# mo-hanxuan/FEMcy

Hardware: AMD Instinct MI355X
Metric: CG iters/sec + element-stiffness assemblies/sec, 1M C3D4 elems, 1/2/4/8 GPU (higher is better)
Workload: dtype f64; 1 GPU; twist plate C3D4 96x12x144 cells, 995328 elements, 548535 DOF (BASELINE configs[2] at N=1, configs[3] at N=8), state S1 (t=0.05), step = assemble K + Dirichlet + 1000 PCG iterations; elements_per_gpu=995328, parallelism=single GPU, launcher=single process

## Files before the change

femcy_amd/backend.py:

```python
from __future__ import annotations

import ctypes as C
import os
from typing import Optional, Sequence

import numpy as np

_HERE = os.path.dirname(os.path.abspath(__file__))
LIB_PATH = os.environ.get("FEMCY_HIP_LIB") or os.path.join(_HERE, "libfemcy_hip.so")
CPU_LIB_PATH = os.environ.get("FEMCY_CPU_LIB") or os.path.join(_HERE, "libfemcy_cpu.so")


def default_backend() -> str:
    kind = os.environ.get("FEMCY_BACKEND", "hip").lower()
    if kind not in ("hip", "cpu"):
        raise FemcyError(f"FEMCY_BACKEND={kind!r}: expected 'hip' or 'cpu'")
    return kind

VEC_DOF, VEC_RHS, VEC_RESIDUAL, VEC_FORCE, VEC_DU, VEC_DOF_OLD, VEC_X, VEC_TMP0, VEC_TMP1 = range(9)
GP_DSDX, GP_VOL, GP_F, GP_SIGMA, GP_STRAIN, GP_MISES, GP_ENERGY = range(7)
OPT_ASSEMBLY, OPT_PCG_POLL, OPT_TIMING, OPT_SPMV_VARIANT, OPT_EW_GRID, OPT_PCG_GRAPH, OPT_SELL_SIGMA = range(7)
OPT_TANGENT = 7
OPT_EXCHANGE = 8
OPT_PCG_STORAGE_ORDER = 13
OPT_PCG_FUSED_UPDATE = 15
OPT_SPMV_FOOTPRINT = 16
OPT_DIRECT_MAX_BYTES = 17
OPT_NODE_ORDER = 14
OPT_PCG_PERSIST = 11
OPT_PCG_PERSIST_MULTI = 12
OPT_PCG_SMALL = 10
TUNE_PERSIST_VARIANT = 109
TUNE_SKIP_OCCUPANCY_CHECK = 111
TUNE_BARRIER_SPIN_LIMIT = 112
TUNE_PERSIST_L2_ROWS = 113
TUNE_SPMV_WG_PER_XCD = 101
TUNE_SPMV_ROT = 119
TUNE_PAIRS = 117
TUNE_DIRECT_UPDATE = 115
TUNE_PERSIST_MAX_MB = 114
OPT_OVERLAP = 9
ASM_GATHER, ASM_ATOMIC, ASM_ROWS, ASM_AUTO, ASM_GATHER_SYM, ASM_GATHER_SYM_ROWSUM, ASM_ROWS2, ASM_ROWS4, ASM_PAIRS = 0, 1, 2, 3, 4, 5, 6, 8, 9
ASM_ROWS3 = 7

EXPORTS = [
    "femcy_ctx_create", "femcy_ctx_destroy", "femcy_last_error", "femcy_version", "femcy_set_option", "femcy_sync",
    "femcy_set_mesh", "femcy_set_element", "femcy_set_material", "femcy_build_pattern", "femcy_get_pattern_info",
    "femcy_get_assembly_used",
    "femcy_vec_upload", "femcy_vec_download", "femcy_vec_fill", "femcy_vec_copy", "femcy_vec_scatter",
    "femcy_vec_sub", "femcy_vec_axpy", "femcy_vec_scale", "femcy_vec_norm", "femcy_vec_absmax",
# ... 510 lines not shown
```

femcy_amd/csrc/ctx.hpp:

```cpp
#pragma once
#include <hip/hip_runtime.h>
#include <stdint.h>
#include <stdlib.h>
#include <mutex>
#include <string>
#include <vector>
#include "../../include/femcy.h"

namespace femcy {

void set_error(const char* fmt, ...);

#define FEMCY_HIP(call)                                                                         \
    do {                                                                                        \
        hipError_t _e = (call);                                                                 \
        if (_e != hipSuccess) {                                                                 \
            femcy::set_error("%s failed: %s (%s:%d)", #call, hipGetErrorString(_e), __FILE__, __LINE__); \
            return FEMCY_EHIP;                                                                  \
        }                                                                                       \
    } while (0)

inline hipError_t dfill_sync(void* p, int value, size_t bytes) {
    if (!bytes) return hipSuccess;
#ifdef FEMCY_TEST_LATE_FILL
// ... 168 lines not shown
    double* d_val_scratch = nullptr;
    int64_t scratch_cap = 0;

    hipGraphExec_t pcg_graph = nullptr;
    const double* pcg_graph_x = nullptr;
    int pcg_graph_iters = 0, pcg_graph_g = 0, pcg_graph_np1 = 0;
    int opt_graph = 1;
    int opt_persist = 1;
    int64_t persist_max_bytes = (int64_t)1 << 40;
    int opt_persist_rj = 4;
    int opt_persist_wgs = 0;
    int opt_persist_l2rows = 1;
    int opt_persist_variant = -1;
    int opt_persist_dbg = 0;
    int opt_persist_lds = -1;
    int persist_cus = 0;
    bool persist_failed = false;
    bool small_failed = false;
    int opt_skip_occupancy = 0;
    uint32_t barrier_spin_limit = 1u << 20;
    int32_t* d_persist_assign = nullptr;
    std::vector<int64_t> persist_assign_key;
    int64_t pattern_serial = 0;
    double* d_persist = nullptr;
    int64_t persist_cap = 0;
    int32_t* d_bcolp = nullptr;
    int64_t bcolp_serial = -1;
    int opt_spmv_fp = 0;
    uint16_t* d_lcol = nullptr;
    int32_t* d_fp_ptr = nullptr;
    int32_t* d_fp = nullptr;
    int32_t fp_cap = 0;
    int64_t fp_serial = -1;
    int opt_fused_update = 0;
    bool fused_failed = false;
    double* d_fused = nullptr;
    int opt_pos_space = 1;
// ... 166 lines not shown
```

femcy_amd/csrc/femcy_api.cpp:

```cpp
#include <algorithm>
#include <cmath>
#include <cstdarg>
#include <chrono>
#include <cstdio>
#include <cstring>
#include "ctx.hpp"
#include "direct.hpp"

namespace femcy {

static thread_local char g_err[1024] = "";

void set_error(const char* fmt, ...) {
    va_list ap;
    va_start(ap, fmt);
    vsnprintf(g_err, sizeof(g_err), fmt, ap);
    va_end(ap);
}

template <class T>
static int dev_alloc(T** p, size_t count, bool zero = true) {
    if (*p) {
        (void)hipFree(*p);
        *p = nullptr;
// ... 291 lines not shown
            break;
        case FEMCY_OPT_EXCHANGE:
            FEMCY_REQUIRE(value == 0 || value == 1, "exchange: 0 (all-reduce) or 1 (neighbour send/recv)");
            FEMCY_REQUIRE(value == 0 || c->d_if_ptr, "femcy_comm_set_neighbours must come first");
            c->exchange = (int)value;
            break;
        case FEMCY_OPT_PCG_PERSIST:
            FEMCY_REQUIRE(value >= 0 && value <= 2, "persistent PCG: 0 (off), 1 (auto) or 2 (whenever the slices fit)");
            c->opt_persist = (int)value;
            c->persist_failed = false;
            break;
        case FEMCY_TUNE_PERSIST_LDS_ROWS:
            FEMCY_REQUIRE(value >= -1 && value <= 64, "resident block rows out of range");
            c->opt_persist_lds = (int)value;
            break;
        case FEMCY_TUNE_SPMV_KEEP:
            FEMCY_REQUIRE(value >= -1 && value <= 1000, "per-mille out of range (-1 = auto)");
            c->opt_spmv_keep = (int)value;
            if (c->have_pattern) {
                pcg_graph_reset(c);
                spmv_split(c);
            }
            break;
        case FEMCY_TUNE_SMALL_REG_ROWS:
            FEMCY_REQUIRE(value >= -1 && value <= 64, "register-resident rows out of range");
            c->opt_small_rr = (int)value;
            break;
        case FEMCY_TUNE_PERSIST_WGS:
            FEMCY_REQUIRE(value >= 0 && value <= 4096, "workgroup count out of range");
            c->opt_persist_wgs = (int)value;
// ... 42 lines not shown
        case FEMCY_TUNE_PERSIST_VARIANT:
            FEMCY_REQUIRE(value >= -1 && value <= 15 && (value < 8 || value == 14), "variant bits: -1 (default), 0..7 or 14");
            c->opt_persist_variant = (int)value;
            break;
        case FEMCY_TUNE_PERSIST_PROBE:
#ifdef FEMCY_PERSIST_PROBE
            c->opt_persist_dbg = (int)value;
            break;
#else
            FEMCY_REQUIRE(value == 0 || value == 16, "option 106: the work-skipping timing switches (bits 0-3) exist only in a "
                                                     "-DFEMCY_PERSIST_PROBE build; 16 (no prefetch during the barriers) is always available");
            c->opt_persist_dbg = (int)value;
            break;
#endif
        case FEMCY_TUNE_PERSIST_REG_ROWS:
#ifdef FEMCY_PERSIST_PIPE
            FEMCY_REQUIRE(value == 0 || value == 2 || value == 4 || value == 5, "register-resident block rows: 0, 2, 4 or 5");
#else
            FEMCY_REQUIRE(value == 0 || value == 4 || value == 5, "register-resident block rows: 0, 4 or 5");
#endif
            c->opt_persist_rj = (int)value;
            break;
        case FEMCY_OPT_PCG_SMALL:
            FEMCY_REQUIRE(value == 0 || value == 1, "small-system PCG: 0 (off) or 1 (auto)");
            c->opt_small = (int)value;
            c->small_failed = false;
            break;
        case FEMCY_OPT_OVERLAP:
            FEMCY_REQUIRE(value == 0 || value == 1, "overlap: 0 (one stream) or 1 (exchange overlapped with the interior product)");
            c->opt_overlap = (int)value;
            break;
        case FEMCY_OPT_TANGENT:
            FEMCY_REQUIRE(value == 0 || value == 1, "tangent: 0 (reference) or 1 (consistent)");
            c->opt_tangent = (int)value;
            break;
// ... 1011 lines not shown
```

femcy_amd/csrc/kernels_pcg_persist.hip:

```cpp
#include <algorithm>
#include <cmath>
#include <type_traits>
#include <vector>
#include "ctx.hpp"
#include "wave_reduce.hpp"
#include "granule.hpp"

#if defined(__HIP_DEVICE_COMPILE__) && !defined(__gfx950__) && !defined(__gfx942__)
#error "k_pcg_persist: the sc1-only hand-off protocol is validated for gfx942 / gfx950 only"
#endif

namespace femcy {

namespace {

constexpr int PBS = 256;
constexpr int PNX = 8;
constexpr int CH = 4;
constexpr int V_NT = 1, V_A2A = 2, V_WIDE = 4, V_INBAND = 8;
constexpr unsigned SENT_HI = 0xFFFBADD0u, SENT_LO = 0x5E471E70u;

#ifdef FEMCY_PERSIST_PROBE
#define PDBG(a_, bit_) ((a_).dbg & (bit_))
#else
#define PDBG(a_, bit_) false
#endif

struct PersistPcg {
    const int32_t* slice_len;
    const int64_t* slice_off;
    const int32_t* bcol;
    const int32_t* node_of;
    const int32_t* assign;
    const double* vals;
    const double* b;
    const double* M;
    double* x;
    double* dbuf;
    double* part1;
    double* part2;
    double* slots;
    unsigned int* xc;
    unsigned int* top;
    PcgState* st;
    int32_t npad, maxit, lds_rows, dbg, l2_rows;
    uint32_t spin_limit;
    uint32_t xspin_limit;
    double eps;
    unsigned long long* mbox;
    unsigned long long* const* peer;
    const int32_t* mr_tab;
    const uint8_t* owner;
    int32_t rank, nranks, nb_total;
    uint32_t tagbase;
};

__device__ __forceinline__ void pst(double* p, double v) {
    __hip_atomic_store(p, v, __ATOMIC_RELAXED, __HIP_MEMORY_SCOPE_AGENT);
}
__device__ __forceinline__ double pld(const double* p) {
// ... 120 lines not shown
    constexpr bool NT = (VAR & V_NT) != 0, A2A = (VAR & V_A2A) != 0, WIDE = (VAR & V_WIDE) != 0;
    constexpr bool INB = (VAR & V_INBAND) != 0;
#ifndef FEMCY_PERSIST_OWN_DIAG
#define FEMCY_PERSIST_OWN_DIAG 1
#endif
    constexpr bool OWN_DIAG = INB || (FEMCY_PERSIST_OWN_DIAG && WIDE);
    static_assert(!INB || (WIDE && A2A), "in-band validity of d is built on the storage-order, tagged-granule form");
    constexpr int NDB = INB ? 3 : 2;
    extern __shared__ __attribute__((aligned(16))) char lds_persist[];
    __shared__ double sm1[PBS / 64], sm2[PBS / 64], bc[2];
    __shared__ int s_fail;
    const int tid = threadIdx.x, lane = tid & 63;
    const int wave = __builtin_amdgcn_readfirstlane(tid >> 6);
    const int G = gridDim.x;
    if (tid == 0) s_fail = 0;
    double* lvals = reinterpret_cast<double*>(lds_persist) + (size_t)wave * a.lds_rows * DD * 64;
    int32_t* lcols = reinterpret_cast<int32_t*>(lds_persist + (size_t)4 * a.lds_rows * DD * 64 * 8) + (size_t)wave * a.lds_rows * 64;

    const int xk = blockIdx.x % PNX;
    const int nwx = (G / PNX) * 4;
    const int wx = (blockIdx.x / PNX) * 4 + wave;
    int32_t sl[SPW], Ls[SPW], node[SPW], dpos[SPW];
    uint32_t inmask = 0;
#define IN(t_) (((inmask >> (t_)) & 1u) != 0)
    int32_t offs32[SPW];
#define OFFS(t_) ((int64_t)offs32[t_])
#pragma unroll
    for (int t = 0; t < SPW; ++t) {
        const int32_t s = __builtin_amdgcn_readfirstlane(a.assign[((size_t)xk * nwx + wx) * SPW + t]);
        const bool act = s >= 0;
        sl[t] = act ? s : -1;
        Ls[t] = act ? __builtin_amdgcn_readfirstlane(a.slice_len[s]) : 0;
// ... 6 lines not shown
    double rv[SPW][RJ > 0 ? RJ : 1][DD];
    int32_t rcl[SPW][RJ > 0 ? RJ : 1];
#pragma unroll
    for (int t = 0; t < SPW; ++t)
#pragma unroll
        for (int jj = 0; jj < RJ; ++jj) {
            const bool has = jj < Ls[t];
            const double* src = a.vals + (OFFS(t) + (has ? jj : 0)) * (int64_t)(DD * 64);
#pragma unroll
            for (int k = 0; k < DD; ++k) rv[t][jj][k] = has ? src[kv_index<DM>(0, k, lane)] : 0.0;
            rcl[t][jj] = has ? a.bcol[(OFFS(t) + jj) * 64 + lane] : dpos[t];
        }
    uint32_t jq[SPW];
#define JL(t_) ((int32_t)(jq[t_] & 0xffu))
#define QL(t_) ((int32_t)((jq[t_] >> 8) & 0xffu))
#define JE(t_) ((int32_t)(jq[t_] >> 16))
    {
        int qn = 0;
#pragma unroll
        for (int t = SPW - 1; t >= 0; --t) {
            const int jl_ = min(RJ, Ls[t]);
            const int nl = max(0, min(Ls[t] - jl_, a.lds_rows - qn));
            jq[t] = (uint32_t)jl_ | ((uint32_t)qn << 8) | ((uint32_t)(jl_ + nl) << 16);
            qn += nl;
            for (int32_t j = JL(t); j < JE(t); ++j) {
                const int q = QL(t) + (j - JL(t));
                const double* src = a.vals + (OFFS(t) + j) * (int64_t)(DD * 64);
#pragma unroll
                for (int k = 0; k < DD; ++k) lvals[(q * DD + k) * 64 + lane] = src[kv_index<DM>(0, k, lane)];
                lcols[q * 64 + lane] = a.bcol[(OFFS(t) + j) * 64 + lane];
            }
        }
    }
    const __amdgpu_buffer_rsrc_t drsrc = __builtin_amdgcn_make_buffer_rsrc(
        (void*)a.dbuf, 0, (int)((size_t)NDB * a.npad * sizeof(double)), 0x00020000);
    auto gather_d = [&](int32_t col, int32_t parity_off, double (&xv)[DM]) {
        if (WIDE) {
            const u32x4 w = __builtin_amdgcn_raw_buffer_load_b128(drsrc, col * (DM * 8), parity_off, AUX_SC1);
            xv[0] = __hiloint2double((int)w.y, (int)w.x);
            xv[1] = __hiloint2double((int)w.w, (int)w.z);
            if (DM == 3) {
                const u32x2 w2 = __builtin_amdgcn_raw_buffer_load_b64(drsrc, col * (DM * 8) + 16, parity_off, AUX_SC1);
                xv[DM - 1] = __hiloint2double((int)w2.y, (int)w2.x);
            }
        } else {
// ... 33 lines not shown
        w.x = SENT_LO; w.y = SENT_HI; w.z = SENT_LO; w.w = SENT_HI;
        __builtin_amdgcn_raw_buffer_store_b128(w, drsrc, p * (DM * 8), buf_off, AUX_SC1);
        if (DM == 3) {
            u32x2 w2;
            w2.x = SENT_LO; w2.y = SENT_HI;
            __builtin_amdgcn_raw_buffer_store_b64(w2, drsrc, p * (DM * 8) + 16, buf_off, AUX_SC1);
        }
    };
    auto stale_d = [&](const double (&xv)[DM]) -> bool {
        bool st = false;
#pragma unroll
        for (int cc = 0; cc < DM; ++cc) st = st || ((unsigned)__double2hiint(xv[cc]) == SENT_HI);
        return st;
    };
    typedef double nt_d2 __attribute__((ext_vector_type(2)));
    auto load_rows = [&](const int32_t* __restrict__ bc_, const double2* __restrict__ vp, const double* __restrict__ vs,
                         int32_t j, int nb, int32_t keep0, int32_t (&col)[CH], double (&e)[CH][DD]) {
#pragma unroll
        for (int u = 0; u < CH; ++u) col[u] = bc_[(int64_t)(j + max(0, min(u, nb - 1))) * 64];
#pragma unroll
        for (int u = 0; u < CH; ++u)
            if (u < nb) {
                if (NT && j + u >= keep0) {
#pragma unroll
                    for (int kp = 0; kp < NP; ++kp) {
                        const nt_d2 v2 = __builtin_nontemporal_load(
                            reinterpret_cast<const nt_d2*>(&vp[(int64_t)(j + u) * (DD * 32) + kp * 64]));
                        e[u][2 * kp] = v2.x;
                        e[u][2 * kp + 1] = v2.y;
                    }
                    if (DD & 1) e[u][DD - 1] = __builtin_nontemporal_load(&vs[(int64_t)(j + u) * (DD * 64)]);
                } else {
#pragma unroll
                    for (int kp = 0; kp < NP; ++kp) {
// ... 7 lines not shown
#pragma unroll
                for (int k = 0; k < DD; ++k) e[u][k] = 0.0;
            }
    };
    const int32_t* __restrict__ bc0 = a.bcol + OFFS(0) * 64 + lane;
    const double2* __restrict__ vp0 = reinterpret_cast<const double2*>(a.vals + OFFS(0) * (int64_t)(DD * 64)) + lane;
    const double* __restrict__ vs0 = a.vals + OFFS(0) * (int64_t)(DD * 64) + NP * 128 + lane;
#ifndef FEMCY_INB_PREFETCH
#define FEMCY_INB_PREFETCH 1
#endif
    constexpr bool PREFETCH = !(DM == 3 && SPW >= 7);
    const int npf = (!PREFETCH || (a.dbg & 16) || (A2A && wave == 0) || (INB && !FEMCY_INB_PREFETCH)) ? 0 : max(0, min(CH, Ls[0] - JE(0)));
    int32_t pcol[CH];
    double pe[CH][DD];
    const int32_t jpf = npf > 0 ? JE(0) : 0;
    if (PREFETCH) load_rows(bc0, vp0, vs0, jpf, npf, JE(0) + a.l2_rows, pcol, pe);
    double xo[SPW][DM], rr[SPW][DM], mm[SPW][DM], dd[SPW][DM], Ad[SPW][DM];
    double accs = 0.0, accm = 0.0;
    uint32_t ownbits = 0;
#pragma unroll
    for (int t = 0; t < SPW; ++t) {
#pragma unroll
        for (int c = 0; c < DM; ++c) {
            const bool in = node[t] >= 0;
            const int64_t i = in ? (int64_t)node[t] * DM + c : 0;
            const double bl = a.b[i], ml = a.M[i];
            const double bi = in ? bl : 0.0, mi = in ? ml : 0.0;
            xo[t][c] = 0.0;
            rr[t][c] = bi;
            mm[t][c] = mi;
            dd[t][c] = mi * bi;
// ... 127 lines not shown
    auto product = [&](const int32_t poff) -> double {
        double acc[SPW][DM];
#pragma unroll
        for (int t = 0; t < SPW; ++t)
#pragma unroll
            for (int r = 0; r < DM; ++r) acc[t][r] = 0.0;
#pragma unroll
        for (int t = 0; t < SPW; ++t) {
            const int32_t L = Ls[t];
            const int32_t* __restrict__ bcp = a.bcol + OFFS(t) * 64 + lane;
            const double2* __restrict__ vp = reinterpret_cast<const double2*>(a.vals + OFFS(t) * (int64_t)(DD * 64)) + lane;
            const double* __restrict__ vs = a.vals + OFFS(t) * (int64_t)(DD * 64) + NP * 128 + lane;
            int32_t j = JE(t);
            if (PREFETCH && t == 0 && npf > 0 && !PDBG(a, 1)) {
                double xg[CH][DM];
#pragma unroll
                for (int u = 0; u < CH; ++u) gather_d(pcol[u], poff, xg[u]);
                __builtin_amdgcn_sched_barrier(0);
                FEMCY_SETTLE(CH, _Pragma("unroll") for (int u = 0; u < CH; ++u) gather_d(pcol[u], poff, xg[u]))
#pragma unroll
                for (int u = 0; u < CH; ++u)
                    if (u < npf) {
#pragma unroll
                        for (int r = 0; r < DM; ++r)
#pragma unroll
                            for (int cc = 0; cc < DM; ++cc) acc[t][r] += pe[u][r * DM + cc] * xg[u][cc];
                    }
                j += npf;
            }
            if (RJ > 0 && !PDBG(a, 4)) {
// ... 32 lines not shown
                double xg[CH][DM];
#pragma unroll
                for (int u = 0; u < CH; ++u) gather_d(lcols[(q + min(u, nb - 1)) * 64 + lane], poff, xg[u]);
                __builtin_amdgcn_sched_barrier(0);
                FEMCY_SETTLE(CH, _Pragma("unroll") for (int u = 0; u < CH; ++u) gather_d(lcols[(q + min(u, nb - 1)) * 64 + lane], poff, xg[u]))
#pragma unroll
                for (int u = 0; u < CH; ++u)
                    if (u < nb) {
#pragma unroll
                        for (int r = 0; r < DM; ++r)
#pragma unroll
                            for (int cc = 0; cc < DM; ++cc)
                                acc[t][r] += lvals[((q + u) * DD + r * DM + cc) * 64 + lane] * xg[u][cc];
                    }
            }
#ifdef FEMCY_PERSIST_PIPE
            if (j < L && !PDBG(a, 1)) {
                int32_t colA[CH], colB[CH];
                double eA[CH][DD], eB[CH][DD];
                int nbA = min(CH, L - j), nbB = 0;
                load_rows(bcp, vp, vs, j, nbA, JE(t) + a.l2_rows, colA, eA);
                for (;;) {
                    {
                        double xg[CH][DM];
#pragma unroll
                        for (int u = 0; u < CH; ++u) gather_d(colA[u], poff, xg[u]);
                        __builtin_amdgcn_sched_barrier(0);
                        const int32_t jn = j + nbA;
                        nbB = max(0, min(CH, L - jn));
                        load_rows(bcp, vp, vs, nbB > 0 ? jn : j, nbB, JE(t) + a.l2_rows, colB, eB);
                        __builtin_amdgcn_sched_barrier(0);
#pragma unroll
                        for (int u = 0; u < CH; ++u)
                            if (u < nbA) {
#pragma unroll
                                for (int r = 0; r < DM; ++r)
#pragma unroll
                                    for (int cc = 0; cc < DM; ++cc) acc[t][r] += eA[u][r * DM + cc] * xg[u][cc];
                            }
                        j = jn;
                        __builtin_amdgcn_sched_barrier(0);
                    }
                    if (nbB == 0) break;
                    {
                        double xg[CH][DM];
#pragma unroll
                        for (int u = 0; u < CH; ++u) gather_d(colB[u], poff, xg[u]);
                        __builtin_amdgcn_sched_barrier(0);
                        const int32_t jn = j + nbB;
                        nbA = max(0, min(CH, L - jn));
                        load_rows(bcp, vp, vs, nbA > 0 ? jn : j, nbA, JE(t) + a.l2_rows, colA, eA);
                        __builtin_amdgcn_sched_barrier(0);
#pragma unroll
                        for (int u = 0; u < CH; ++u)
                            if (u < nbB) {
#pragma unroll
                                for (int r = 0; r < DM; ++r)
#pragma unroll
                                    for (int cc = 0; cc < DM; ++cc) acc[t][r] += eB[u][r * DM + cc] * xg[u][cc];
                            }
                        j = jn;
                        __builtin_amdgcn_sched_barrier(0);
                    }
                    if (nbA == 0) break;
                }
            }
#endif
            while (j < L && !PDBG(a, 1)) {
                const int nb = min(CH, L - j);
                int32_t col[CH];
                double e[CH][DD], xg[CH][DM];
                load_rows(bcp, vp, vs, j, nb, JE(t) + a.l2_rows, col, e);
#pragma unroll
                for (int u = 0; u < CH; ++u) gather_d(col[u], poff, xg[u]);
                __builtin_amdgcn_sched_barrier(0);
                FEMCY_SETTLE(CH, _Pragma("unroll") for (int u = 0; u < CH; ++u) gather_d(col[u], poff, xg[u]))
#pragma unroll
                for (int u = 0; u < CH; ++u)
                    if (u < nb) {
#pragma unroll
                        for (int r = 0; r < DM; ++r)
#pragma unroll
                            for (int cc = 0; cc < DM; ++cc) acc[t][r] += e[u][r * DM + cc] * xg[u][cc];
                    }
                j += nb;
            }
        }
        double dot = 0.0;
#pragma unroll
// ... 44 lines not shown
                double o[1];
                const int op[1] = {0};
                const bool okx = granule_sweep<1>(srsrc, 0, G, tag, a.spin_limit, o, op);
                if (!okx) poison_granules();
                if (lane == 0) {
                    bc[0] = o[0];
                    if (!okx) s_fail = 1;
                }
#pragma unroll
                for (int u = 0; u < CH; ++u) {
                    pcol[u] = 0;
#pragma unroll
                    for (int k = 0; k < DD; ++k) pe[u][k] = 0.0;
                }
            } else if (PREFETCH) {
                load_rows(bc0, vp0, vs0, jpf, npf, JE(0) + a.l2_rows, pcol, pe);
            }
            ++round;
            __syncthreads();
            if (s_fail) { done = 3; return; }
            dAd = bc[0];
        } else {
            if (tid == 0) pst(a.part1 + (size_t)(it & 1) * G + blockIdx.x, (sm1[0] + sm1[1]) + (sm1[2] + sm1[3]));
            if (!grid_barrier(a, round++, &s_fail, [&] { if (PREFETCH) load_rows(bc0, vp0, vs0, jpf, npf, JE(0) + a.l2_rows, pcol, pe); })) { done = 3; return; }
            double ps = 0.0;
            for (int k = tid; k < G; k += PBS) ps += pld(a.part1 + (size_t)(it & 1) * G + k);
            ps = wave_sum(ps);
            __syncthreads();
            if (lane == 0) sm1[wave] = ps;
            __syncthreads();
            dAd = (sm1[0] + sm1[1]) + (sm1[2] + sm1[3]);
        }
        if (MULTI) {
            double val[1] = {dAd};
            const int op[1] = {0};
            if (!xrank_stage(std::integral_constant<int, 1>{}, MB_SA, val, op)) { done = 3; return; }
            dAd = val[0];
            const uint32_t tag = mb_tag(a.tagbase, it);
            bool okr = true;
// ... 88 lines not shown
            for (int c = 0; c < DM; ++c) a.x[nd * DM + c] = xo[t][c];
        }
    if (blockIdx.x == 0 && tid == 0) {
        a.st->iters = it;
        a.st->r0 = r0;
        a.st->rmax = rmax;
        a.st->done = done;
        a.st->rMr[0] = rMr;
    }
}
#undef IN
#undef OFFS
#undef JL
#undef QL
#undef JE

template <int U>
__global__ void __launch_bounds__(PBS) k_probe_stream(const double2* __restrict__ buf, int64_t n16, int reps, int nt,
                                                      double* __restrict__ sink) {
    const int G = gridDim.x, xk = blockIdx.x % PNX, per = G / PNX;
    const int64_t chunk = (n16 / G) / (PBS * U) * (PBS * U);
    double s0 = 0.0, s1 = 0.0;
    typedef double nt_d2 __attribute__((ext_vector_type(2)));
    for (int r = 0; r < reps; ++r) {
        const int64_t wg = (int64_t)xk * per + (blockIdx.x / PNX + (int64_t)r * (per / 3 + 1)) % per;
        const double2* __restrict__ p = buf + wg * chunk + threadIdx.x;
        for (int64_t i = 0; i < chunk; i += PBS * U) {
            double2 v[U];
#pragma unroll
            for (int u = 0; u < U; ++u) {
// ... 145 lines not shown
    hipLaunchKernelGGL(k_bcol_to_pos, dim3((unsigned)((nb + 255) / 256)), dim3(256), 0, c->stream, nb,
                       (const int32_t*)c->d_bcol, (const int32_t*)c->d_pos, c->d_bcolp);
    FEMCY_HIP(hipGetLastError());
    c->bcolp_serial = c->pattern_serial;
    return FEMCY_OK;
}

#ifndef FEMCY_PERSIST_DEFAULT_VARIANT
#define FEMCY_PERSIST_DEFAULT_VARIANT 6
#endif

constexpr int PERSIST_MULTI_RETRY = 16;

int64_t persist_streamed_bytes(Ctx* c);

struct PersistShape { int G, nwx, SPW, rj, lds_rows; int32_t maxrange; };
bool persist_shape(const Ctx* c, PersistShape* out) {
    PersistShape sh{};
    sh.G = ((c->opt_persist_wgs > 0 ? c->opt_persist_wgs : c->persist_cus) / PNX) * PNX;
    if (sh.G < PNX || !c->have_pattern) return false;
    sh.nwx = (sh.G / PNX) * 4;
    sh.maxrange = 0;
    for (int k = 0; k < PNX; ++k) sh.maxrange = std::max(sh.maxrange, c->xcd.start[k + 1] - c->xcd.start[k]);
    const int per_wave = (sh.maxrange + sh.nwx - 1) / sh.nwx;
    const bool on = c->opt_persist_rj != 0;
    if (c->dm == 3) {
        if (per_wave > 7) return false;
        sh.SPW = per_wave > 3 ? per_wave : 3;
        if (const char* e = getenv("FEMCY_DEBUG_FORCE_SPW")) sh.SPW = std::min(7, std::max(sh.SPW, atoi(e)));
        sh.rj = sh.SPW == 3 ? c->opt_persist_rj : (!on ? 0 : (sh.SPW == 4 ? 3 : (sh.SPW == 7 ? 0 : 1)));
    } else {
        if (per_wave > 8) return false;
        sh.SPW = per_wave > 6 ? 8 : (per_wave > 4 ? 6 : (per_wave > 3 ? 4 : 3));
        sh.rj = !on ? 0 : (sh.SPW == 8 ? 2 : (sh.SPW == 6 ? 3 : 5));
    }
    const int DD = c->dm * c->dm;
    int lds_rows = c->opt_persist_lds < 0 ? (int)((c->small_max_lds - 2048) / (4 * 64 * (DD * 8 + 4))) : c->opt_persist_lds;
    sh.lds_rows = std::max(0, std::min(lds_rows, sh.SPW * (int)c->max_row_blocks));
    *out = sh;
    return true;
}

bool persist_pattern_fits(Ctx* c) {
    if (!c->opt_persist || !c->have_pattern) return false;
    PersistShape sh;
    if (!persist_shape(c, &sh) || (c->dm == 3 && sh.SPW > 4)) return false;
    const int G = sh.G;
    if (c->opt_persist >= 2) return true;
    if (c->nslices < G / 2) return false;
    const int64_t limit = std::min<int64_t>(c->persist_max_bytes, (int64_t)240 << 20);
    const int64_t row_bytes = (int64_t)(c->dm * c->dm * 8 + 4) * 64;
    return c->stored_rows * row_bytes <= limit || persist_streamed_bytes(c) <= limit;
}

// ... 7 lines not shown
            c->persist_multi_fallbacks = 0;
        }
    }
    if (multi && (!c->persist_multi || c->persist_multi_failed || !c->opt_persist_multi)) return FEMCY_OK;
    PersistShape sh;
    if (!persist_shape(c, &sh)) return FEMCY_OK;
    const int G = sh.G, nwx = sh.nwx;
    if ((c->nslices < G + G / 2) && c->opt_persist < 2 && !multi) return FEMCY_OK;
    const int DD = c->dm * c->dm;
    const int SPW = sh.SPW, lds_rows = sh.lds_rows;
    const int rj = sh.rj;
    const int64_t row_bytes = (int64_t)(DD * 8 + 4) * 64;
    const int64_t kbytes = c->stored_rows * row_bytes;
    const int64_t resident = (int64_t)G * 4 * (SPW * rj + lds_rows) * row_bytes;
    if (kbytes - resident > c->persist_max_bytes && c->opt_persist < 2 && !multi) return FEMCY_OK;
    const size_t lds = (size_t)4 * lds_rows * 64 * (DD * 8 + 4) + 16;
    const int var = c->opt_persist_variant < 0 ? FEMCY_PERSIST_DEFAULT_VARIANT : c->opt_persist_variant;
    const bool wide = (var & V_WIDE) != 0, a2a = (var & V_A2A) != 0;
    const int64_t npad = wide ? (((int64_t)c->nslices * SLICE * c->dm + 1) & ~(int64_t)1) : ((c->n + 1) & ~(int64_t)1);
    size_t tp = (size_t)-1;
    bool launched = true, not_resident = false;
    auto setup_and_launch = [&]() -> int {
        PersistPcg a;
        {
            int rc = persist_buffers(c, G, npad, &a);
            if (rc) return rc;
        }
        {
            std::vector<int64_t> key = {G, SPW, c->pattern_serial, a2a ? 1 : 0};
            for (int k = 0; k <= PNX; ++k) key.push_back(c->xcd.start[k]);
            if (key != c->persist_assign_key || !c->d_persist_assign) {
                std::vector<int32_t> assign((size_t)PNX * nwx * SPW, -1);
                std::vector<int32_t> order, load(nwx), cnt(nwx);
                for (int k = 0; k < PNX; ++k) {
                    order.clear();
                    for (int32_t s = c->xcd.start[k]; s < c->xcd.start[k + 1]; ++s) order.push_back(s);
                    std::stable_sort(order.begin(), order.end(),
                                     [&](int32_t x, int32_t y) { return c->h_slice_len[x] > c->h_slice_len[y]; });
                    for (int w = 0; w < nwx; ++w) load[w] = (a2a && (w % 4) == 0) ? CH : 0;
                    std::fill(cnt.begin(), cnt.end(), 0);
                    for (int32_t s : order) {
                        int best = -1;
                        for (int w = 0; w < nwx; ++w)
                            if (cnt[w] < SPW && (best < 0 || load[w] < load[best])) best = w;
                        assign[((size_t)k * nwx + best) * SPW + cnt[best]++] = s;
                        load[best] += c->h_slice_len[s];
                    }
                }
                if (c->d_persist_assign) (void)hipFree(c->d_persist_assign);
                c->d_persist_assign = nullptr;
                FEMCY_HIP(dmalloc(&c->d_persist_assign, assign.size() * sizeof(int32_t)));
                FEMCY_HIP(hipMemcpyAsync(c->d_persist_assign, assign.data(), assign.size() * sizeof(int32_t),
                                         hipMemcpyHostToDevice, c->stream));
                FEMCY_HIP(hipStreamSynchronize(c->stream));
                c->persist_assign_key = key;
            }
        }
        if (wide) {
            int rc = ensure_bcolp(c);
            if (rc) return rc;
        }
        a.assign = c->d_persist_assign;
        a.slice_len = c->d_slice_len; a.slice_off = c->d_slice_off; a.bcol = wide ? c->d_bcolp : c->d_bcol; a.node_of = c->d_node_of;
        a.vals = c->d_Kvals; a.b = d_b; a.M = c->d_M; a.x = d_x;
        a.st = c->d_state;
        a.npad = (int32_t)npad; a.maxit = maxit; a.lds_rows = lds_rows; a.eps = eps;
        a.l2_rows = c->opt_persist_l2rows;
        a.mbox = c->d_mbox; a.peer = c->d_peer_tab; a.mr_tab = c->d_mr_tab; a.owner = c->d_owner;
        a.rank = c->rank; a.nranks = c->nranks; a.nb_total = c->h_nb_ptr.empty() ? 0 : c->h_nb_ptr.back();
        c->solve_serial = (c->solve_serial % 4095) + 1;
        a.tagbase = c->solve_serial << 20;
#define FEMCY_PERSIST_M(DM_, SPW_, RJ_, VAR_, MULTI_)                                                             \
        do {                                                                                                          \
            const void* fn = reinterpret_cast<const void*>(&k_pcg_persist<DM_, SPW_, RJ_, VAR_, MULTI_>);             \
            if (lds > 48 * 1024)                                                                                      \
                FEMCY_HIP(hipFuncSetAttribute(fn, hipFuncAttributeMaxDynamicSharedMemorySize, (int)lds));             \
             \
             \
            if (!coresident(c, fn, PBS, lds, G)) {                                                                    \
                not_resident = true;                                                                                  \
                launched = false;                                                                                     \
// ... 31 lines not shown
            if (c->dm == 3) {
                FEMCY_REQUIRE(SPW <= 4, "the multi-rank persistent PCG of 3 x 3 blocks exists for up to four slices per wave");
                if (SPW == 3) { FEMCY_PERSIST_M(3, 3, 4, FEMCY_PERSIST_DEFAULT_VARIANT, true); }
                else { FEMCY_PERSIST_M(3, 4, 3, FEMCY_PERSIST_DEFAULT_VARIANT, true); }
            } else if (SPW == 3) { FEMCY_PERSIST_M(2, 3, 5, FEMCY_PERSIST_DEFAULT_VARIANT, true); }
            else if (SPW == 4) { FEMCY_PERSIST_M(2, 4, 5, FEMCY_PERSIST_DEFAULT_VARIANT, true); }
            else if (SPW == 6) { FEMCY_PERSIST_M(2, 6, 3, FEMCY_PERSIST_DEFAULT_VARIANT, true); }
            else { FEMCY_PERSIST_M(2, 8, 2, FEMCY_PERSIST_DEFAULT_VARIANT, true); }
        } else
#ifdef FEMCY_PERSIST_ONLY_334
        if (c->dm == 3 && SPW == 3 && c->opt_persist_rj == 4) { FEMCY_PERSIST_V(3, 3, 4) } else return FEMCY_OK;
#else
        if (c->dm == 3 && SPW == 3) {
            if (c->opt_persist_rj == 5) { FEMCY_PERSIST_V(3, 3, 5) }
            else if (c->opt_persist_rj == 4) { FEMCY_PERSIST_V(3, 3, 4) }
#ifdef FEMCY_PERSIST_PIPE
            else if (c->opt_persist_rj == 2) { FEMCY_PERSIST_V(3, 3, 2) }
#endif
            else { FEMCY_PERSIST_V(3, 3, 0) }
        } else if (c->dm == 3 && SPW == 4) {
            if (c->opt_persist_rj) { FEMCY_PERSIST_V(3, 4, 3) } else { FEMCY_PERSIST_V(3, 4, 0) }
        } else if (c->dm == 3) {
            FEMCY_REQUIRE((var & 15) == FEMCY_PERSIST_DEFAULT_VARIANT, "5 .. 7 slices per wave exist for the default variant of the persistent PCG only");
            if (SPW == 5) { if (c->opt_persist_rj) FEMCY_PERSIST(3, 5, 1, FEMCY_PERSIST_DEFAULT_VARIANT); else FEMCY_PERSIST(3, 5, 0, FEMCY_PERSIST_DEFAULT_VARIANT); }
            else if (SPW == 6) { if (c->opt_persist_rj) FEMCY_PERSIST(3, 6, 1, FEMCY_PERSIST_DEFAULT_VARIANT); else FEMCY_PERSIST(3, 6, 0, FEMCY_PERSIST_DEFAULT_VARIANT); }
            else { FEMCY_PERSIST(3, 7, 0, FEMCY_PERSIST_DEFAULT_VARIANT); }
        } else if (SPW == 3) {
            if (c->opt_persist_rj) { FEMCY_PERSIST_V(2, 3, 5) } else { FEMCY_PERSIST_V(2, 3, 0) }
        } else if (SPW == 4) {
            if (c->opt_persist_rj) { FEMCY_PERSIST_V(2, 4, 5) } else { FEMCY_PERSIST_V(2, 4, 0) }
        } else if (SPW == 6) {
            if (c->opt_persist_rj) { FEMCY_PERSIST_V(2, 6, 3) } else { FEMCY_PERSIST_V(2, 6, 0) }
        } else {
// ... 174 lines not shown
    }
    if (rc == FEMCY_EHIP) set_error("probe_mailbox: a HIP call failed: %s", hipGetErrorString(hipGetLastError()));
    if (rc) return rc;
    *us_per_round = ticks / (double)khz * 1e3 / rounds;
    return FEMCY_OK;
}

int64_t persist_streamed_bytes(Ctx* c) {
    PersistShape sh;
    if (!persist_shape(c, &sh) || c->nslices < sh.G) return 0;
    const int G = sh.G, DD = c->dm * c->dm, lds_rows = sh.lds_rows, rj = sh.rj;
    const int64_t row_bytes = (int64_t)(DD * 8 + 4) * 64;
    int64_t reg_rows = 0;
    for (int32_t s = 0; s < c->nslices; ++s) reg_rows += std::min<int64_t>(c->h_slice_len[s], rj);
    const int64_t lds_total = std::min<int64_t>((int64_t)G * 4 * lds_rows, c->stored_rows - reg_rows);
    return (c->stored_rows - reg_rows - lds_total) * row_bytes;
}

}
```

femcy_amd/csrc_cpu/femcy_cpu.cpp:

```cpp
#include <omp.h>
#include <algorithm>
#include <chrono>
#include <cmath>
#include <cstdarg>
#include <cstdio>
#include <cstring>
#include <new>
#include <vector>
#include "../../include/femcy.h"
#include "../csrc/band_order.hpp"
#include "../csrc/element_math.hpp"

using namespace femcy;

namespace {

thread_local char g_err[1024] = "";
void set_error(const char* fmt, ...) {
    va_list ap;
    va_start(ap, fmt);
    vsnprintf(g_err, sizeof(g_err), fmt, ap);
    va_end(ap);
}
#define REQUIRE(cond, ...)          \
// ... 353 lines not shown
        case FEMCY_OPT_SELL_SIGMA:
            REQUIRE(!c->have_pattern, "set the sorting window before femcy_build_pattern");
            return FEMCY_OK;
        case FEMCY_OPT_ASSEMBLY: case FEMCY_OPT_PCG_POLL: case FEMCY_OPT_SPMV_VARIANT: case FEMCY_OPT_EW_GRID:
        case FEMCY_OPT_PCG_GRAPH: case FEMCY_OPT_PCG_PERSIST: case FEMCY_OPT_PCG_SMALL: case FEMCY_OPT_OVERLAP:
        case FEMCY_OPT_PCG_PERSIST_MULTI: case FEMCY_OPT_PCG_STORAGE_ORDER: case FEMCY_OPT_PCG_FUSED_UPDATE: case FEMCY_OPT_SPMV_FOOTPRINT:
            return FEMCY_OK;
        case FEMCY_OPT_NODE_ORDER:
            REQUIRE(!c->have_pattern, "set the node order before femcy_build_pattern");
            return FEMCY_OK;
        case FEMCY_OPT_DIRECT_MAX_BYTES:
            REQUIRE(value >= (int64_t)1 << 20, "direct solve: the band limit must be at least 1 MiB");
            c->direct_max_bytes = value;
            return FEMCY_OK;
        default:
            if (option >= 100 && option <= 119) return FEMCY_OK;
            set_error("unknown option %d", option);
            return FEMCY_EINVAL;
    }
}
int femcy_sync(femcy_ctx* ctx) {
    CTX_OR_FAIL(ctx);
    (void)c;
    return FEMCY_OK;
}

int femcy_set_mesh(femcy_ctx* ctx, int32_t nn, int32_t dm, const double* nodes, int32_t ne, int32_t npe,
                   const int32_t* elems) {
    CTX_OR_FAIL(ctx);
    REQUIRE(nodes && elems, "null mesh arrays");
    REQUIRE(nn > 0 && ne > 0, "empty mesh (nn=%d, ne=%d)", nn, ne);
// ... 867 lines not shown
```

include/femcy.h:

```cpp
#ifndef FEMCY_H
#define FEMCY_H

#include <stdint.h>

#ifdef __cplusplus
extern "C" {
#endif

typedef struct femcy_ctx femcy_ctx;

enum femcy_status {
    FEMCY_OK = 0,
    FEMCY_EINVAL = -1,
    FEMCY_EHIP = -2,
    FEMCY_ENOKERNEL = -3,
    FEMCY_ENUMERIC = -4,
    FEMCY_ECOMM = -5,
    FEMCY_ENOMEM = -6
};

enum femcy_vec {
    FEMCY_VEC_DOF = 0,
    FEMCY_VEC_RHS = 1,
    FEMCY_VEC_RESIDUAL = 2,
// ... 50 lines not shown
    FEMCY_OPT_PCG_FUSED_UPDATE = 15,
    FEMCY_OPT_SPMV_FOOTPRINT = 16,
    FEMCY_OPT_DIRECT_MAX_BYTES = 17,
    FEMCY_OPT_NODE_ORDER = 14,
    FEMCY_OPT_PCG_PERSIST = 11,
    FEMCY_OPT_PCG_PERSIST_MULTI = 12,
    FEMCY_OPT_PCG_SMALL = 10,
    FEMCY_OPT_OVERLAP = 9,
    FEMCY_OPT_TANGENT = 7,

    FEMCY_TUNE_TIMING_FENCE = 100,
    FEMCY_TUNE_SPMV_WG_PER_XCD = 101,
    FEMCY_TUNE_SPMV_NT = 102,
    FEMCY_TUNE_VEC_NT = 103,
    FEMCY_TUNE_PERSIST_LDS_ROWS = 104,
    FEMCY_TUNE_PERSIST_REG_ROWS = 105,
    FEMCY_TUNE_PERSIST_PROBE = 106,
    FEMCY_TUNE_PERSIST_WGS = 107,
    FEMCY_TUNE_SMALL_REG_ROWS = 108,
    FEMCY_TUNE_PERSIST_VARIANT = 109,
    FEMCY_TUNE_SPMV_KEEP = 110,
    FEMCY_TUNE_SKIP_OCCUPANCY_CHECK = 111,
    FEMCY_TUNE_PERSIST_L2_ROWS = 113,
    FEMCY_TUNE_DIRECT_UPDATE = 115,
    FEMCY_TUNE_SPMV_ROT = 119,
    FEMCY_TUNE_PAIRS = 117,
    FEMCY_TUNE_PERSIST_MAX_MB = 114,
    FEMCY_TUNE_BARRIER_SPIN_LIMIT = 112
};

// ... 124 lines not shown
```

Measured before the change: 36690 CG iters/s x (global elements / 995328).

## Cache streamed SpMV column indices in LDS for persistent PCG kernel

Adds an LDS-resident column-index table per wave in the persistent PCG kernel, so the streamed block rows read their column indices from LDS instead of global memory. The x gather can then be issued before the value loads. A host-side planner trades resident value rows against column-table rows under the LDS budget, and slice assignment is hoisted into a reusable host helper. The change also removes the experimental FEMCY_PERSIST_PIPE double-buffer path. The cost is more LDS per workgroup, which may reduce the value rows that stay resident, plus a more complex prefetch path.

```diff
diff --git a/femcy_amd/backend.py b/femcy_amd/backend.py
--- a/femcy_amd/backend.py
+++ b/femcy_amd/backend.py
@@ -34,6 +34,7 @@
 TUNE_SKIP_OCCUPANCY_CHECK = 111
 TUNE_BARRIER_SPIN_LIMIT = 112
 TUNE_PERSIST_L2_ROWS = 113
+TUNE_PERSIST_COL_ROWS = 120
 TUNE_SPMV_WG_PER_XCD = 101
 TUNE_SPMV_ROT = 119
 TUNE_PAIRS = 117
diff --git a/femcy_amd/csrc/ctx.hpp b/femcy_amd/csrc/ctx.hpp
--- a/femcy_amd/csrc/ctx.hpp
+++ b/femcy_amd/csrc/ctx.hpp
@@ -206,6 +206,7 @@
     int opt_persist_variant = -1;
     int opt_persist_dbg = 0;
     int opt_persist_lds = -1;
+    int opt_persist_cols = -1;
     int persist_cus = 0;
     bool persist_failed = false;
     bool small_failed = false;
@@ -213,6 +214,10 @@
     uint32_t barrier_spin_limit = 1u << 20;
     int32_t* d_persist_assign = nullptr;
     std::vector<int64_t> persist_assign_key;
+    std::vector<int32_t> h_persist_assign;
+    std::vector<int64_t> h_persist_assign_key;
+    std::vector<int64_t> persist_layout_key;
+    int persist_layout_lds = 0, persist_layout_cols = 0;
     int64_t pattern_serial = 0;
     double* d_persist = nullptr;
     int64_t persist_cap = 0;
diff --git a/femcy_amd/csrc/femcy_api.cpp b/femcy_amd/csrc/femcy_api.cpp
--- a/femcy_amd/csrc/femcy_api.cpp
+++ b/femcy_amd/csrc/femcy_api.cpp
@@ -329,6 +329,10 @@
             FEMCY_REQUIRE(value >= -1 && value <= 64, "resident block rows out of range");
             c->opt_persist_lds = (int)value;
             break;
+        case FEMCY_TUNE_PERSIST_COL_ROWS:
+            FEMCY_REQUIRE(value >= -1 && value <= 200, "column-table rows: -1 (auto), 0 (off) or a cap of 1 .. 200");
+            c->opt_persist_cols = (int)value;
+            break;
         case FEMCY_TUNE_SPMV_KEEP:
             FEMCY_REQUIRE(value >= -1 && value <= 1000, "per-mille out of range (-1 = auto)");
             c->opt_spmv_keep = (int)value;
@@ -401,11 +405,7 @@
             break;
 #endif
         case FEMCY_TUNE_PERSIST_REG_ROWS:
-#ifdef FEMCY_PERSIST_PIPE
-            FEMCY_REQUIRE(value == 0 || value == 2 || value == 4 || value == 5, "register-resident block rows: 0, 2, 4 or 5");
-#else
             FEMCY_REQUIRE(value == 0 || value == 4 || value == 5, "register-resident block rows: 0, 4 or 5");
-#endif
             c->opt_persist_rj = (int)value;
             break;
         case FEMCY_OPT_PCG_SMALL:
diff --git a/femcy_amd/csrc/kernels_pcg_persist.hip b/femcy_amd/csrc/kernels_pcg_persist.hip
--- a/femcy_amd/csrc/kernels_pcg_persist.hip
+++ b/femcy_amd/csrc/kernels_pcg_persist.hip
@@ -25,6 +25,10 @@
 #else
 #define PDBG(a_, bit_) false
 #endif
+
+constexpr bool persist_col_table(int dm, int spw, int rj, int var, bool multi) {
+    return !(dm == 3 && (rj == 5 || (spw == 4 && rj == 3) || (spw == 3 && rj == 4 && ((var & 8) != 0 || multi))));
+}
 
 struct PersistPcg {
     const int32_t* slice_len;
@@ -44,6 +48,7 @@
     unsigned int* top;
     PcgState* st;
     int32_t npad, maxit, lds_rows, dbg, l2_rows;
+    int32_t col_rows;
     uint32_t spin_limit;
     uint32_t xspin_limit;
     double eps;
@@ -194,8 +199,11 @@
     const int wave = __builtin_amdgcn_readfirstlane(tid >> 6);
     const int G = gridDim.x;
     if (tid == 0) s_fail = 0;
+    constexpr bool COLTAB = persist_col_table(DM, SPW, RJ, VAR, MULTI);
+    const int32_t ncol = COLTAB ? a.col_rows : 0;
     double* lvals = reinterpret_cast<double*>(lds_persist) + (size_t)wave * a.lds_rows * DD * 64;
     int32_t* lcols = reinterpret_cast<int32_t*>(lds_persist + (size_t)4 * a.lds_rows * DD * 64 * 8) + (size_t)wave * a.lds_rows * 64;
+    int32_t* ccols = reinterpret_cast<int32_t*>(lds_persist + (size_t)4 * a.lds_rows * 64 * (DD * 8 + 4)) + (size_t)wave * ncol * 64;
 
     const int xk = blockIdx.x % PNX;
     const int nwx = (G / PNX) * 4;
@@ -232,7 +240,8 @@
     uint32_t jq[SPW];
 #define JL(t_) ((int32_t)(jq[t_] & 0xffu))
 #define QL(t_) ((int32_t)((jq[t_] >> 8) & 0xffu))
-#define JE(t_) ((int32_t)(jq[t_] >> 16))
+#define JE(t_) ((int32_t)(COLTAB ? (jq[t_] >> 16) & 0xffu : jq[t_] >> 16))
+#define CB(t_) ((int32_t)(jq[t_] >> 24))
     {
         int qn = 0;
 #pragma unroll
@@ -247,6 +256,17 @@
 #pragma unroll
                 for (int k = 0; k < DD; ++k) lvals[(q * DD + k) * 64 + lane] = src[kv_index<DM>(0, k, lane)];
                 lcols[q * 64 + lane] = a.bcol[(OFFS(t) + j) * 64 + lane];
+            }
+        }
+        if (COLTAB) {
+            int cn = 0;
+#pragma unroll
+            for (int t = 0; t < SPW; ++t) {
+                jq[t] |= (uint32_t)min(cn, 255) << 24;
+                const int ns = max(0, Ls[t] - JE(t));
+                for (int i = 0; i < ns && cn + i < ncol; ++i)
+                    ccols[(cn + i) * 64 + lane] = a.bcol[(OFFS(t) + JE(t) + i) * 64 + lane];
+                cn += ns;
             }
         }
     }
@@ -310,10 +330,16 @@
         return st;
     };
     typedef double nt_d2 __attribute__((ext_vector_type(2)));
-    auto load_rows = [&](const int32_t* __restrict__ bc_, const double2* __restrict__ vp, const double* __restrict__ vs,
-                         int32_t j, int nb, int32_t keep0, int32_t (&col)[CH], double (&e)[CH][DD]) {
+    auto table_cols = [&](int nb, int32_t cq, int32_t (&col)[CH]) {
+#pragma unroll
+        for (int u = 0; u < CH; ++u) col[u] = ccols[(cq + max(0, min(u, nb - 1))) * 64 + lane];
+    };
+    auto load_cols = [&](const int32_t* __restrict__ bc_, int32_t j, int nb, int32_t (&col)[CH]) {
 #pragma unroll
         for (int u = 0; u < CH; ++u) col[u] = bc_[(int64_t)(j + max(0, min(u, nb - 1))) * 64];
+    };
+    auto load_vals = [&](const double2* __restrict__ vp, const double* __restrict__ vs, int32_t j, int nb, int32_t keep0,
+                         double (&e)[CH][DD]) {
 #pragma unroll
         for (int u = 0; u < CH; ++u)
             if (u < nb) {
@@ -351,7 +377,17 @@
     int32_t pcol[CH];
     double pe[CH][DD];
     const int32_t jpf = npf > 0 ? JE(0) : 0;
-    if (PREFETCH) load_rows(bc0, vp0, vs0, jpf, npf, JE(0) + a.l2_rows, pcol, pe);
+    const bool pf_tab = COLTAB && npf > 0 && npf <= ncol;
+    auto load_prefetch = [&]() {
+        if (pf_tab) {
+#pragma unroll
+            for (int u = 0; u < CH; ++u) pcol[u] = 0;
+        } else {
+            load_cols(bc0, jpf, npf, pcol);
+        }
+        load_vals(vp0, vs0, jpf, npf, JE(0) + a.l2_rows, pe);
+    };
+    if (PREFETCH) load_prefetch();
     double xo[SPW][DM], rr[SPW][DM], mm[SPW][DM], dd[SPW][DM], Ad[SPW][DM];
     double accs = 0.0, accm = 0.0;
     uint32_t ownbits = 0;
@@ -509,6 +545,7 @@
             int32_t j = JE(t);
             if (PREFETCH && t == 0 && npf > 0 && !PDBG(a, 1)) {
                 double xg[CH][DM];
+                if (pf_tab) table_cols(npf, 0, pcol);
 #pragma unroll
                 for (int u = 0; u < CH; ++u) gather_d(pcol[u], poff, xg[u]);
                 __builtin_amdgcn_sched_barrier(0);
@@ -571,65 +608,25 @@
                                 acc[t][r] += lvals[((q + u) * DD + r * DM + cc) * 64 + lane] * xg[u][cc];
                     }
             }
-#ifdef FEMCY_PERSIST_PIPE
-            if (j < L && !PDBG(a, 1)) {
-                int32_t colA[CH], colB[CH];
-                double eA[CH][DD], eB[CH][DD];
-                int nbA = min(CH, L - j), nbB = 0;
-                load_rows(bcp, vp, vs, j, nbA, JE(t) + a.l2_rows, colA, eA);
-                for (;;) {
-                    {
-                        double xg[CH][DM];
-#pragma unroll
-                        for (int u = 0; u < CH; ++u) gather_d(colA[u], poff, xg[u]);
-                        __builtin_amdgcn_sched_barrier(0);
-                        const int32_t jn = j + nbA;
-                        nbB = max(0, min(CH, L - jn));
-                        load_rows(bcp, vp, vs, nbB > 0 ? jn : j, nbB, JE(t) + a.l2_rows, colB, eB);
-                        __builtin_amdgcn_sched_barrier(0);
-#pragma unroll
-                        for (int u = 0; u < CH; ++u)
-                            if (u < nbA) {
-#pragma unroll
-                                for (int r = 0; r < DM; ++r)
-#pragma unroll
-                                    for (int cc = 0; cc < DM; ++cc) acc[t][r] += eA[u][r * DM + cc] * xg[u][cc];
-                            }
-                        j = jn;
-                        __builtin_amdgcn_sched_barrier(0);
-                    }
-                    if (nbB == 0) break;
-                    {
-                        double xg[CH][DM];
-#pragma unroll
-                        for (int u = 0; u < CH; ++u) gather_d(colB[u], poff, xg[u]);
-                        __builtin_amdgcn_sched_barrier(0);
-                        const int32_t jn = j + nbB;
-                        nbA = max(0, min(CH, L - jn));
-                        load_rows(bcp, vp, vs, nbA > 0 ? jn : j, nbA, JE(t) + a.l2_rows, colA, eA);
-                        __builtin_amdgcn_sched_barrier(0);
-#pragma unroll
-                        for (int u = 0; u < CH; ++u)
-                            if (u < nbB) {
-#pragma unroll
-                                for (int r = 0; r < DM; ++r)
-#pragma unroll
-                                    for (int cc = 0; cc < DM; ++cc) acc[t][r] += eB[u][r * DM + cc] * xg[u][cc];
-                            }
-                        j = jn;
-                        __builtin_amdgcn_sched_barrier(0);
-                    }
-                    if (nbA == 0) break;
-                }
-            }
-#endif
             while (j < L && !PDBG(a, 1)) {
                 const int nb = min(CH, L - j);
+                const int32_t cq = CB(t) + (j - JE(t));
                 int32_t col[CH];
                 double e[CH][DD], xg[CH][DM];
-                load_rows(bcp, vp, vs, j, nb, JE(t) + a.l2_rows, col, e);
-#pragma unroll
-                for (int u = 0; u < CH; ++u) gather_d(col[u], poff, xg[u]);
+                const bool tab = COLTAB && cq + nb <= ncol;
+                if (tab) {
+                    table_cols(nb, cq, col);
+#pragma unroll
+                    for (int u = 0; u < CH; ++u) gather_d(col[u], poff, xg[u]);
+                    __builtin_amdgcn_sched_barrier(0);
+                } else {
+                    load_cols(bcp, j, nb, col);
+                }
+                load_vals(vp, vs, j, nb, JE(t) + a.l2_rows, e);
+                if (!tab) {
+#pragma unroll
+                    for (int u = 0; u < CH; ++u) gather_d(col[u], poff, xg[u]);
+                }
                 __builtin_amdgcn_sched_barrier(0);
                 FEMCY_SETTLE(CH, _Pragma("unroll") for (int u = 0; u < CH; ++u) gather_d(col[u], poff, xg[u]))
 #pragma unroll
@@ -704,7 +701,7 @@
                     for (int k = 0; k < DD; ++k) pe[u][k] = 0.0;
                 }
             } else if (PREFETCH) {
-                load_rows(bc0, vp0, vs0, jpf, npf, JE(0) + a.l2_rows, pcol, pe);
+                load_prefetch();
             }
             ++round;
             __syncthreads();
@@ -712,7 +709,7 @@
             dAd = bc[0];
         } else {
             if (tid == 0) pst(a.part1 + (size_t)(it & 1) * G + blockIdx.x, (sm1[0] + sm1[1]) + (sm1[2] + sm1[3]));
-            if (!grid_barrier(a, round++, &s_fail, [&] { if (PREFETCH) load_rows(bc0, vp0, vs0, jpf, npf, JE(0) + a.l2_rows, pcol, pe); })) { done = 3; return; }
+            if (!grid_barrier(a, round++, &s_fail, [&] { if (PREFETCH) load_prefetch(); })) { done = 3; return; }
             double ps = 0.0;
             for (int k = tid; k < G; k += PBS) ps += pld(a.part1 + (size_t)(it & 1) * G + k);
             ps = wave_sum(ps);
@@ -831,6 +828,7 @@
 #undef JL
 #undef QL
 #undef JE
+#undef CB
 
 template <int U>
 __global__ void __launch_bounds__(PBS) k_probe_stream(const double2* __restrict__ buf, int64_t n16, int reps, int nt,
@@ -1006,8 +1004,35 @@
 
 int64_t persist_streamed_bytes(Ctx* c);
 
-struct PersistShape { int G, nwx, SPW, rj, lds_rows; int32_t maxrange; };
-bool persist_shape(const Ctx* c, PersistShape* out) {
+struct PersistShape { int G, nwx, SPW, rj, lds_rows, col_rows; int32_t maxrange; };
+
+static std::vector<int64_t> persist_assign_host(Ctx* c, int G, int nwx, int SPW, bool a2a) {
+    std::vector<int64_t> key = {G, SPW, c->pattern_serial, a2a ? 1 : 0};
+    for (int k = 0; k <= PNX; ++k) key.push_back(c->xcd.start[k]);
+    if (key == c->h_persist_assign_key) return key;
+    std::vector<int32_t> assign((size_t)PNX * nwx * SPW, -1);
+    std::vector<int32_t> order, load(nwx), cnt(nwx);
+    for (int k = 0; k < PNX; ++k) {
+        order.clear();
+        for (int32_t s = c->xcd.start[k]; s < c->xcd.start[k + 1]; ++s) order.push_back(s);
+        std::stable_sort(order.begin(), order.end(),
+                         [&](int32_t x, int32_t y) { return c->h_slice_len[x] > c->h_slice_len[y]; });
+        for (int w = 0; w < nwx; ++w) load[w] = (a2a && (w % 4) == 0) ? CH : 0;
+        std::fill(cnt.begin(), cnt.end(), 0);
+        for (int32_t s : order) {
+            int best = -1;
+            for (int w = 0; w < nwx; ++w)
+                if (cnt[w] < SPW && (best < 0 || load[w] < load[best])) best = w;
+            assign[((size_t)k * nwx + best) * SPW + cnt[best]++] = s;
+            load[best] += c->h_slice_len[s];
+        }
+    }
+    c->h_persist_assign.swap(assign);
+    c->h_persist_assign_key = key;
+    return key;
+}
+
+static bool persist_shape_base(const Ctx* c, PersistShape* out) {
     PersistShape sh{};
     sh.G = ((c->opt_persist_wgs > 0 ? c->opt_persist_wgs : c->persist_cus) / PNX) * PNX;
     if (sh.G < PNX || !c->have_pattern) return false;
@@ -1019,7 +1044,8 @@
     if (c->dm == 3) {
         if (per_wave > 7) return false;
         sh.SPW = per_wave > 3 ? per_wave : 3;
-        if (const char* e = getenv("FEMCY_DEBUG_FORCE_SPW")) sh.SPW = std::min(7, std::max(sh.SPW, atoi(e)));
+        static const int force_spw = [] { const char* e = getenv("FEMCY_DEBUG_FORCE_SPW"); return e ? atoi(e) : 0; }();
+        if (force_spw) sh.SPW = std::min(7, std::max(sh.SPW, force_spw));
         sh.rj = sh.SPW == 3 ? c->opt_persist_rj : (!on ? 0 : (sh.SPW == 4 ? 3 : (sh.SPW == 7 ? 0 : 1)));
     } else {
         if (per_wave > 8) return false;
@@ -1029,7 +1055,53 @@
     const int DD = c->dm * c->dm;
     int lds_rows = c->opt_persist_lds < 0 ? (int)((c->small_max_lds - 2048) / (4 * 64 * (DD * 8 + 4))) : c->opt_persist_lds;
     sh.lds_rows = std::max(0, std::min(lds_rows, sh.SPW * (int)c->max_row_blocks));
+    sh.col_rows = 0;
     *out = sh;
+    return true;
+}
+
+bool persist_shape(Ctx* c, PersistShape* out) {
+    PersistShape sh;
+    if (!persist_shape_base(c, &sh)) return false;
+    *out = sh;
+    const int var = c->opt_persist_variant < 0 ? FEMCY_PERSIST_DEFAULT_VARIANT : c->opt_persist_variant;
+    if (c->opt_persist_cols == 0 || !persist_col_table(c->dm, sh.SPW, sh.rj, var & 15, c->comm != nullptr)) return true;
+    std::vector<int64_t> key = persist_assign_host(c, sh.G, sh.nwx, sh.SPW, (var & V_A2A) != 0);
+    key.insert(key.end(), {sh.rj, sh.lds_rows, c->opt_persist_lds, c->opt_persist_cols, (int64_t)c->small_max_lds, c->dm});
+    if (key != c->persist_layout_key) {
+        const int DD = c->dm * c->dm;
+        const int64_t vrow = (int64_t)4 * 64 * (DD * 8 + 4), crow = (int64_t)4 * 64 * 4;
+        const int64_t avail = std::max<int64_t>(c->small_max_lds - 2048, sh.lds_rows * vrow);
+        const int cap = c->opt_persist_cols < 0 ? 200 : std::min(200, c->opt_persist_cols);
+        std::vector<int32_t> rows((size_t)PNX * sh.nwx, 0);
+        for (size_t w = 0; w < rows.size(); ++w)
+            for (int t = 0; t < sh.SPW; ++t) {
+                const int32_t s = c->h_persist_assign[w * sh.SPW + t];
+                if (s >= 0) rows[w] += std::max(0, c->h_slice_len[s] - sh.rj);
+            }
+        const int32_t longest = rows.empty() ? 0 : *std::max_element(rows.begin(), rows.end());
+        int best_l = sh.lds_rows, best_c = 0;
+        int64_t best_bytes = -1;
+        bool best_cov = false;
+        for (int l = sh.lds_rows; l >= (c->opt_persist_lds < 0 ? std::max(0, sh.lds_rows - 1) : sh.lds_rows); --l) {
+            const int need = std::max(0, longest - l);
+            const int cr = (int)std::min<int64_t>(std::min(cap, need), (avail - l * vrow) / crow);
+            const bool cov = cr >= need;
+            int64_t bytes = 0;
+            for (int32_t r : rows) {
+                const int64_t st = std::max(0, r - l);
+                bytes += st * (DD * 8) * 64 + std::max<int64_t>(0, st - cr) * 4 * 64;
+            }
+            if (best_bytes < 0 || (cov && !best_cov) || (cov == best_cov && bytes < best_bytes)) {
+                best_l = l; best_c = cr; best_bytes = bytes; best_cov = cov;
+            }
+        }
+        c->persist_layout_lds = best_l;
+        c->persist_layout_cols = best_c;
+        c->persist_layout_key = key;
+    }
+    out->lds_rows = c->persist_layout_lds;
+    out->col_rows = c->persist_layout_cols;
     return true;
 }
 
@@ -1067,7 +1139,7 @@
     const int64_t kbytes = c->stored_rows * row_bytes;
     const int64_t resident = (int64_t)G * 4 * (SPW * rj + lds_rows) * row_bytes;
     if (kbytes - resident > c->persist_max_bytes && c->opt_persist < 2 && !multi) return FEMCY_OK;
-    const size_t lds = (size_t)4 * lds_rows * 64 * (DD * 8 + 4) + 16;
+    const size_t lds = (size_t)4 * lds_rows * 64 * (DD * 8 + 4) + (size_t)4 * sh.col_rows * 64 * 4 + 16;
     const int var = c->opt_persist_variant < 0 ? FEMCY_PERSIST_DEFAULT_VARIANT : c->opt_persist_variant;
     const bool wide = (var & V_WIDE) != 0, a2a = (var & V_A2A) != 0;
     const int64_t npad = wide ? (((int64_t)c->nslices * SLICE * c->dm + 1) & ~(int64_t)1) : ((c->n + 1) & ~(int64_t)1);
@@ -1080,26 +1152,9 @@
             if (rc) return rc;
         }
         {
-            std::vector<int64_t> key = {G, SPW, c->pattern_serial, a2a ? 1 : 0};
-            for (int k = 0; k <= PNX; ++k) key.push_back(c->xcd.start[k]);
+            const std::vector<int64_t> key = persist_assign_host(c, G, nwx, SPW, a2a);
             if (key != c->persist_assign_key || !c->d_persist_assign) {
-                std::vector<int32_t> assign((size_t)PNX * nwx * SPW, -1);
-                std::vector<int32_t> order, load(nwx), cnt(nwx);
-                for (int k = 0; k < PNX; ++k) {
-                    order.clear();
-                    for (int32_t s = c->xcd.start[k]; s < c->xcd.start[k + 1]; ++s) order.push_back(s);
-                    std::stable_sort(order.begin(), order.end(),
-                                     [&](int32_t x, int32_t y) { return c->h_slice_len[x] > c->h_slice_len[y]; });
-                    for (int w = 0; w < nwx; ++w) load[w] = (a2a && (w % 4) == 0) ? CH : 0;
-                    std::fill(cnt.begin(), cnt.end(), 0);
-                    for (int32_t s : order) {
-                        int best = -1;
-                        for (int w = 0; w < nwx; ++w)
-                            if (cnt[w] < SPW && (best < 0 || load[w] < load[best])) best = w;
-                        assign[((size_t)k * nwx + best) * SPW + cnt[best]++] = s;
-                        load[best] += c->h_slice_len[s];
-                    }
-                }
+                const std::vector<int32_t>& assign = c->h_persist_assign;
                 if (c->d_persist_assign) (void)hipFree(c->d_persist_assign);
                 c->d_persist_assign = nullptr;
                 FEMCY_HIP(dmalloc(&c->d_persist_assign, assign.size() * sizeof(int32_t)));
@@ -1117,7 +1172,7 @@
         a.slice_len = c->d_slice_len; a.slice_off = c->d_slice_off; a.bcol = wide ? c->d_bcolp : c->d_bcol; a.node_of = c->d_node_of;
         a.vals = c->d_Kvals; a.b = d_b; a.M = c->d_M; a.x = d_x;
         a.st = c->d_state;
-        a.npad = (int32_t)npad; a.maxit = maxit; a.lds_rows = lds_rows; a.eps = eps;
+        a.npad = (int32_t)npad; a.maxit = maxit; a.lds_rows = lds_rows; a.col_rows = sh.col_rows; a.eps = eps;
         a.l2_rows = c->opt_persist_l2rows;
         a.mbox = c->d_mbox; a.peer = c->d_peer_tab; a.mr_tab = c->d_mr_tab; a.owner = c->d_owner;
         a.rank = c->rank; a.nranks = c->nranks; a.nb_total = c->h_nb_ptr.empty() ? 0 : c->h_nb_ptr.back();
@@ -1179,9 +1234,6 @@
         if (c->dm == 3 && SPW == 3) {
             if (c->opt_persist_rj == 5) { FEMCY_PERSIST_V(3, 3, 5) }
             else if (c->opt_persist_rj == 4) { FEMCY_PERSIST_V(3, 3, 4) }
-#ifdef FEMCY_PERSIST_PIPE
-            else if (c->opt_persist_rj == 2) { FEMCY_PERSIST_V(3, 3, 2) }
-#endif
             else { FEMCY_PERSIST_V(3, 3, 0) }
         } else if (c->dm == 3 && SPW == 4) {
             if (c->opt_persist_rj) { FEMCY_PERSIST_V(3, 4, 3) } else { FEMCY_PERSIST_V(3, 4, 0) }
@@ -1386,7 +1438,9 @@
     int64_t reg_rows = 0;
     for (int32_t s = 0; s < c->nslices; ++s) reg_rows += std::min<int64_t>(c->h_slice_len[s], rj);
     const int64_t lds_total = std::min<int64_t>((int64_t)G * 4 * lds_rows, c->stored_rows - reg_rows);
-    return (c->stored_rows - reg_rows - lds_total) * row_bytes;
-}
-
-}
+    const int64_t streamed = c->stored_rows - reg_rows - lds_total;
+    const int64_t col_total = std::min<int64_t>((int64_t)G * 4 * sh.col_rows, streamed);
+    return streamed * row_bytes - col_total * 4 * 64;
+}
+
+}
diff --git a/femcy_amd/csrc_cpu/femcy_cpu.cpp b/femcy_amd/csrc_cpu/femcy_cpu.cpp
--- a/femcy_amd/csrc_cpu/femcy_cpu.cpp
+++ b/femcy_amd/csrc_cpu/femcy_cpu.cpp
@@ -391,7 +391,7 @@
             c->direct_max_bytes = value;
             return FEMCY_OK;
         default:
-            if (option >= 100 && option <= 119) return FEMCY_OK;
+            if (option >= 100 && option <= 120) return FEMCY_OK;
             set_error("unknown option %d", option);
             return FEMCY_EINVAL;
     }
diff --git a/include/femcy.h b/include/femcy.h
--- a/include/femcy.h
+++ b/include/femcy.h
@@ -88,6 +88,7 @@
     FEMCY_TUNE_SPMV_NT = 102,
     FEMCY_TUNE_VEC_NT = 103,
     FEMCY_TUNE_PERSIST_LDS_ROWS = 104,
+    FEMCY_TUNE_PERSIST_COL_ROWS = 120,
     FEMCY_TUNE_PERSIST_REG_ROWS = 105,
     FEMCY_TUNE_PERSIST_PROBE = 106,
     FEMCY_TUNE_PERSIST_WGS = 107,
```

After: 34670 CG iters/s x (global elements / 995328). 5.5% lower.
